# AlanLiangC/PDM-SSD

Measured on AMD Instinct MI355X. Metric: frames/sec (16384-pt clouds, bs=32), higher is better.
Workload: dtype f32; 1 GPU; configs[2]: full PDM-SSD forward (PointNet2MSG backbone + PDM neck + hybrid head: BEV heat-map head + point box head with decoded boxes), bs=32/GPU x 16384 pts, uniform KITTI-range clouds, fp32 inference, inputs resident in HBM, 4 distinct batches in rotation; launch=hipGraph, parallelism=dp1, global_batch=32

## Files before the change

### include/pdmssd_hip.h

```cpp
#ifndef PDMSSD_HIP_H
#define PDMSSD_HIP_H

#include <stddef.h>

#ifdef __cplusplus
extern "C" {
#endif

#define PDM_ABI_VERSION 1

#define PDM_E_BADARG (-1)
#define PDM_E_TOOLARGE (-2)

int pdm_abi_version(void);
const char *pdm_last_error(void);


int pdm_ball_query(void *stream, int b, int n, int m, float radius, int nsample,
                   const float *new_xyz, const float *xyz, int *idx);

int pdm_group_points(void *stream, int b, int c, int n, int npoints, int nsample,
                     const float *points, const int *idx, float *out);

int pdm_group_points_grad(void *stream, int b, int c, int n, int npoints, int nsample,
// ... 339 lines not shown
                            const float *V2C, const float *R0, const float *P2, const int *image_shape, long long capacity,
                            int *out_counts, int *overflow, float *out_rows, void *workspace, size_t workspace_bytes);
int pdm_kitti_data_boxes_count(void *stream, int B, int C, long long total_rows, const float *raw, const int *counts,
                               const float *V2C, const float *R0, const float *P2, const int *image_shape, int M,
                               const float *boxes, const int *box_count, int *num_points_in_gt, int *db_count,
                               long long *totals, void *workspace, size_t workspace_bytes);
int pdm_kitti_data_boxes_fill(void *stream, int B, int C, long long total_rows, const float *raw, const int *counts,
                              const float *V2C, const float *R0, const float *P2, const int *image_shape, int M,
                              const float *boxes, const int *box_count, const double *centres, int *num_points_in_gt,
                              int *db_count, long long *totals, long long capacity_points, long long capacity_entries,
                              float *out_points, long long *out_offsets, float *out_boxes, void *workspace,
                              size_t workspace_bytes);

int pdm_interp_concat_rows(void *stream, int b, int n, int m, int c2, int c1, int ld, const void *known, int known_bf16,
                           const void *skip, int skip_bf16, const int *idx, const float *weight, void *out);
int pdm_interp_concat_rows_grad(void *stream, int b, int n, int m, int c2, int ld, const void *dx, const int *idx,
                                const float *weight, float *dknown, void *workspace, size_t workspace_bytes);
int pdm_interp_concat_rows_grad_out(void *stream, int b, int n, int m, int c2, int ld, const void *dx, const int *idx,
                                    const float *weight, void *dknown, int out_bf16, void *workspace, size_t workspace_bytes);

int pdm_tg_stats_parts(long long rows, int N);
int pdm_tg_gemm_nt(void *stream, long long R, int K, int N, const void *X, long long ldx, const void *W, long long ldw,
                   void *Y, long long ldy, const float *bias, float *stats, const float *x_bn_coef);
int pdm_tg_gemm_nt_dy(void *stream, long long R, int K, int N, const void *dZ, long long lddz, const void *Yp, long long ldyp,
                      const void *W, long long ldw, void *dX, long long lddx, void *dYout, long long lddy, const float *coef,
                      const float *grads);
int pdm_tg_gemm_nt_bs(void *stream, long long R, int K, int N, const void *X, long long ldx, const void *W, long long ldw,
                      void *Y, long long ldy, const void *Bx, long long ldbx, const float *bcoef, float *bstats);
int pdm_tg_gemm_nt_pool(void *stream, long long R, int K, int N, const void *X, long long ldx, const void *W, long long ldw,
                        void *Y, long long ldy, const float *bias, float *stats, const float *x_bn_coef, int ns, void *xmax,
                        void *xmin, unsigned char *imax, unsigned char *imin);
int pdm_tg_dy_stats_parts(long long rows, int N);
int pdm_tg_gemm_nt_dy_bs(void *stream, long long R, int K, int N, const void *dZ, long long lddz, const void *Yp, long long ldyp,
                         const void *W, long long ldw, void *dX, long long lddx, void *dYout, long long lddy, const float *coef,
                         const float *grads, const void *Bx, long long ldbx, const float *bcoef, float *bstats);
size_t pdm_tg_wgrad_ws_bytes(long long R, int K, int N);
int pdm_tg_wgrad(void *stream, long long R, int K, int N, const void *dY, long long ldy, const void *X, long long ldx, float *dW,
                 int accumulate, void *workspace, size_t workspace_bytes, const float *x_bn_coef);
size_t pdm_tg_colsum_ws_floats(long long R, int N);
int pdm_tg_colsum(void *stream, long long R, int N, const void *Y, long long ld, float *out, float *scratch);
int pdm_tg_pack_weight(void *stream, int N, int K, const float *W, void *Wb, int ldb, void *Wt, int ldt);
int pdm_tg_pack_weight_pair(void *stream, int N, int K, const float *W, void *Wb, void *Wt, int rows_to, int cols_to);
int pdm_tg_pack_weight_many(void *stream, int njobs, const void *jobs, long long total_blocks);


int pdm_tune_fps_variant(int v);
int pdm_tune_fused_waves(int w);
int pdm_tune_fused_tiles(int t);
int pdm_tune_fused_groups(int n);
int pdm_tune_fused_wg_per_cu(int n);
int pdm_tune_fused_lds_cap(int bytes);
int pdm_tune_fused_reg(int on);
int pdm_tune_fused_gemm(int on);
int pdm_tune_fused_chain(int on);
int pdm_tune_fused_swz(int on);
int pdm_tune_bq_quad(int form);
int pdm_tune_bq_dense_ppc(int hundredths);
int pdm_tune_grid_split(int min_n);
int pdm_tune_bq_small_waves(int w);
int pdm_tune_bq_cpw(int centres);
int pdm_tune_bq_heavy(int candidates);
int pdm_tune_group_lds_floor(int bytes);
int pdm_tune_group_rows(int packed);
int pdm_tune_rows_chain_wg_per_cu(int n);
int pdm_tune_fp_head_tiles(int n);
int pdm_tune_rows_chain_dw_wg_per_cu(int n);
int pdm_tune_rows_chain_xcd(int on);
int pdm_tune_fp_chain_pad_lds(int bytes);
int pdm_tune_fp_chain_nt(int on);
int pdm_tune_fp_chain_mask(int m);
int pdm_tune_group_nt(int on);
int pdm_tune_copy_variant(int v);
int pdm_tune_copy_max_wg(int n);

int pdm_copy_many(void *stream, int count, void *const *dst, const void *const *src, const size_t *bytes);
int pdm_copy_many_dyn(void *stream, int count, void *const *dst, const void *const *src, const size_t *bytes,
                      const int *const *dyn_count, const unsigned *dyn_unit);


int pdm_scatter_bev(void *stream, int B, int P, int C, int degree, const float *xyz,
                    const float *feat, const float *sh, const float *inv2s2, float ox, float oy,
                    float oz, float cx, float cy, float cz, float icx, float icy, float icz, int W,
                    int H, int D, int kx, int ky, int kz, int layout, float *grid, float *wsum);

int pdm_bev_normalize(void *stream, int B, int C, int W, int H, int D, int layout, float eps,
                      float *grid, const float *wsum);

size_t pdm_gather_bev_workspace_bytes(int B, int P, int W, int H, int kx, int ky);
int pdm_gather_bev(void *stream, int B, int P, int C, int degree, const float *xyz, const float *feat,
                   const float *sh, const float *inv2s2, float ox, float oy, float oz, float cx, float cy,
                   float cz, float icx, float icy, float icz, int W, int H, int D, int kx, int ky, int kz,
                   int normalize, float eps, float *grid, float *wsum, void *workspace, size_t workspace_bytes);

int pdm_bev_normalize_grad(void *stream, int B, int C, int W, int H, int D, float eps, const float *y,
                           const float *wsum, const float *dy, float *dx, float *dwsum);

int pdm_scatter_bev_grad(void *stream, int B, int P, int C, int degree, const float *xyz,
                         const float *feat, const float *sh, const float *inv2s2, float ox,
                         float oy, float oz, float cx, float cy, float cz, float icx, float icy,
                         float icz, int W, int H, int D, int kx, int ky, int kz, int layout,
                         const float *dgrid, const float *dwsum, float *dfeat, float *dsh,
                         float *dinv2s2);
int pdm_scatter_bev_grad_normalized(void *stream, int B, int P, int C, int degree, const float *xyz,
                                    const float *feat, const float *sh, const float *inv2s2, float ox,
                                    float oy, float oz, float cx, float cy, float cz, float icx, float icy,
                                    float icz, int W, int H, int D, int kx, int ky, int kz, int layout,
// ... 67 lines not shown
```

### pdm_ssd_amd/csrc/fused_mlp.hip

```cpp
#include "common.h"

#include <mutex>
#include <set>

namespace pdm {

typedef float f4 __attribute__((ext_vector_type(4)));

constexpr int FM_MAXL = 4;

struct MlpDesc {
    int nlayers;
    int K[FM_MAXL + 1];
    int woff[FM_MAXL];
    int boff[FM_MAXL];
    int stage_in;
    int pool_floats;
    int relu_last;
    int lds_p, lds_q;
    int swz;
};

__device__ __forceinline__ int lds_col(int blk, int g, int pos, int swz) {
    const int q = 4 * blk + g;
// ... 931 lines not shown
    for (int unit = wave_id; unit < npairs; unit += nwaves) {
        f4 in[NT];
        int ctr[NT], L[NT];
#pragma unroll
        for (int t = 0; t < NT; ++t) {
            const int2 e = e_next[t];
            ctr[t] = e.y;
            L[t] = pack_tile_L((unit * 2 + t) * 16, m1, m2, m3, m4, m5);
            in[t] = sa_reg_gather(a, (size_t)e.x, a.new_xyz + (size_t)(e.y >= 0 ? e.y : 0) * 3, g);
        }
        {
            const int nunit = unit + nwaves;
#pragma unroll
            for (int t = 0; t < NT; ++t) e_next[t] = pack[nunit < npairs ? (nunit * 2 + t) * 16 + pos : 0];
        }
        f4 h2[NT][B2];
        sa_reg_hidden<B1, B2, NT>(A1, A2, bias1, bias2, in, h2);
        const bool pair = L[0] >= 32;
        float *orow[NT];
#pragma unroll
        for (int t = 0; t < NT; ++t) {
            const int Lw = L[t] < 16 ? L[t] : 16;
            const bool writer = ctr[t] >= 0 && (pos & (Lw - 1)) == 0 && !(pair && t == 1);
            orow[t] = writer ? a.out + (size_t)ctr[t] * a.out_stride + a.out_coff : nullptr;
        }
#pragma unroll
        for (int mb = 0; mb < B3; ++mb) {
            const f4 bi = *reinterpret_cast<const f4 *>(bias3 + 16 * mb);
            f4 v[NT];
#pragma unroll
            for (int t = 0; t < NT; ++t) {
                f4 acc = bi;
#pragma unroll
                for (int kb = 0; kb < B2; ++kb) acc = mfma4(acc, A3[mb][kb], h2[t][kb]);
                v[t] = floor4(acc, 0.0f);
            }
            if (pair) {
                v[0].x = fmaxf(v[0].x, v[1].x); v[0].y = fmaxf(v[0].y, v[1].y);
                v[0].z = fmaxf(v[0].z, v[1].z); v[0].w = fmaxf(v[0].w, v[1].w);
                v[0] = seg_max_nonneg4(v[0], 16);
            } else {
#pragma unroll
                for (int t = 0; t < NT; ++t) v[t] = seg_max_nonneg4(v[t], L[t]);
            }
#pragma unroll
            for (int t = 0; t < NT; ++t)
                if (orow[t]) sa_reg_store4(orow[t], 16 * mb + 4 * g, a.cout, v[t]);
        }
    }
}

int rows_gemm_launch(void *stream, int rows, int cin, const float *in_pm, int k0, int c1, const float *wpack,
                     const float *bias, int relu_last, float *out_pm, int out_stride, int cout);
int rows_chain_launch(void *stream, int rows, int cin, const float *in_pm, int nlayers, const int *dims, const float *wpack,
                      const float *bias, int relu_last, float *out_pm, int out_stride, int cout, int *launched);
int rows_chain_pair_launch(void *stream, int rows, int cin, const float *in_pm, int nlayers, const int *dims, const float *wpack_a,
                           const float *bias_a, const float *wpack_b, const float *bias_b, int relu_last, float *out_a, int out_stride_a,
                           int cout_a, float *out_b, int out_stride_b, int cout_b, int *launched);
static int g_fused_chain = 1;
static int g_fused_pair = 1;
int fp_chain_launch(void *stream, int b, int n, int m, int c_skip, const float *z_pm, int z_stride, const float *skip_pm,
                    const int *idx, const float *weight, const int *dims, const float *wpack, const float *bias, float *out_pm,
                    int out_stride, int cout, int *launched);
int fp_pre_gemm_launch(void *stream, int b, int n, int m, int c_skip, const float *z_pm, int z_stride,
                       const float *skip_pm, const int *idx, const float *weight, int k1, int c2,
                       const float *wpack, const float *bias, float *out_pm, int out_stride, int cout);
static int g_fused_swz = 1;
static int g_fused_gemm = 1;
static int g_fused_reg = 1;
static int g_fused_waves = 0;
static int g_fused_tiles = 0;
static int g_fused_groups = 0;
static int g_fused_lds_cap = 152 * 1024;
static int g_fused_wg_per_cu = 32;

static int fill_desc(const char *who, MlpDesc &d, int nlayers, const int *dims, int k0_real_max, int pool_floats,
                     long long ntiles, int *waves, int *tiles_per_wg, int *groups, bool two_tiles) {
    PDM_REQUIRE(nlayers >= 1 && nlayers <= FM_MAXL, PDM_E_BADARG, "%s: nlayers=%d not in [1,%d]", who, nlayers, FM_MAXL);
    PDM_REQUIRE(dims, PDM_E_BADARG, "%s: null dims", who);
    d.nlayers = nlayers;
    d.relu_last = 1;
    int wo = 0, bo = 0;
    for (int l = 0; l <= nlayers; ++l) {
        PDM_REQUIRE(dims[l] > 0 && dims[l] % 16 == 0, PDM_E_BADARG, "%s: padded width %d of level %d is not a positive multiple of 16", who, dims[l], l);
        d.K[l] = dims[l];
    }
    for (int l = 0; l < nlayers; ++l) {
        d.woff[l] = wo; d.boff[l] = bo;
        wo += d.K[l] * d.K[l + 1];
        bo += d.K[l + 1];
    }
    PDM_REQUIRE(d.K[0] >= k0_real_max, PDM_E_BADARG, "%s: padded input width %d < %d real channels", who, d.K[0], k0_real_max);
    int q = 0, p = 0;
    for (int l = 1; l < nlayers; ++l) {
        if (l & 1) q = q > d.K[l] ? q : d.K[l]; else p = p > d.K[l] ? p : d.K[l];
    }
    int maxmb = 0;
    for (int l = 1; l <= nlayers; ++l) maxmb = maxmb > (d.K[l] >> 4) ? maxmb : (d.K[l] >> 4);
    const int W = g_fused_waves > 0 ? g_fused_waves : maxmb >= 24 ? 8 : maxmb >= 12 ? 4 : maxmb >= 6 ? 2 : 1;
    *waves = W;
    const int p_staged = p > d.K[0] ? p : d.K[0];
    int NT = (W >= 4 && (g_fused_tiles == 2 || (g_fused_tiles == 0 && two_tiles))) ? 2 : 1;
    (void)ntiles;
    auto roww = [](int k) { return g_fused_swz ? (k + 63) / 64 * 64 : k + 4; };
    if ((NT * 16 * (roww(p) + roww(q)) + pool_floats) * 4 > g_fused_lds_cap) NT = 1;
    *tiles_per_wg = NT;
    const int budget = (W == 1 ? 20 : W == 2 ? 40 : W == 4 ? 52 : 64) * 1024;
    d.stage_in = (NT * 16 * (roww(p_staged) + roww(q)) + pool_floats) * 4 <= budget ? 1 : 0;
    if (d.stage_in) p = p_staged;
    d.swz = g_fused_swz;
    d.lds_p = roww(p);
    d.lds_q = roww(q);
    d.pool_floats = pool_floats;
    const int region_bytes = (NT * 16 * (d.lds_p + d.lds_q) + pool_floats) * 4;
    int G = NT == 2 ? 1 : (g_fused_groups > 0 ? g_fused_groups : W == 2 ? 2 : 1);
    while (G > 1 && (G * W > 8 || (long long)G * region_bytes > 64 * 1024 || (long long)G * NT * 4 > ntiles)) G >>= 1;
    *groups = G;
// ... 202 lines not shown
                "sa_mlp_packed_pair: null table");
    PDM_REQUIRE((pack[0] && meta[0] && pack[1] && meta[1]) || b == 0 || m == 0, PDM_E_BADARG, "sa_mlp_packed_pair: null row list");
    SaPlan pl[2];
    for (int k = 0; k < 2; ++k)
        if (int rc = sa_plan(b, n, m, z_pm ? 0 : cin, nsample[k], xyz, new_xyz, z_pm ? nullptr : feat_pm, z_pm, z_stride, z_coff[k], nullptr,
                             nlayers[k], dims[k], wpack[k], bias[k], out_pm, out_stride, out_coff[k], cout[k], pack[k], meta[k], pl[k])) return rc;
    if (b == 0 || m == 0) return 0;
    const bool same = g_sa_pair && !pl[0].reg && !pl[1].reg && pl[0].W == pl[1].W && pl[0].NT == pl[1].NT && pl[0].G == pl[1].G &&
                      pl[0].pre_form == pl[1].pre_form && pl[0].packed && pl[1].packed;
    if (!same) {
        for (int k = 0; k < 2; ++k)
            if (int rc = pdm_sa_mlp_packed(stream, b, n, m, cin, nsample[k], xyz, new_xyz, feat_pm, z_pm, z_stride, z_coff[k], pack[k], meta[k],
                                           nlayers[k], dims[k], wpack[k], bias[k], out_pm, out_stride, out_coff[k], cout[k])) return rc;
        return 0;
    }
    const int W = pl[0].W, NT = pl[0].NT, G = pl[0].G;
    const bool pre_form = pl[0].pre_form;
    const size_t lds_bytes = pl[0].lds_bytes > pl[1].lds_bytes ? pl[0].lds_bytes : pl[1].lds_bytes;
    const dim3 blocks((unsigned)(pl[0].blocks > pl[1].blocks ? pl[0].blocks : pl[1].blocks), 2);
    const SaScale s0{pl[0].d, pl[0].a, pl[0].pack2, meta[0], wpack[0], bias[0]}, s1{pl[1].d, pl[1].a, pl[1].pack2, meta[1], wpack[1], bias[1]};
    FUSED_DISPATCH(sa_packed_pair_kernel, W, G, blocks, lds_bytes, s0, s1);
    return check_launch("sa_mlp_packed_pair");
}

static int fp_fused_launch(void *stream, int mode, int relu_last, int b, int n, int m, int c_known, int c_skip,
                           const float *known_pm, const float *z_pm, int z_stride, const float *skip_pm,
                           const int *idx, const float *weight, int nlayers, const int *dims,
                           const float *wpack, const float *bias, float *out_pm, int out_stride, int cout) {
    PDM_REQUIRE(b >= 0 && n >= 0 && m >= 1 && c_known >= 0 && c_skip >= 0 && c_known + c_skip >= (mode == 1 ? 0 : 1),
                PDM_E_BADARG, "fp_mlp_fused: bad size");
    if (b == 0 || n == 0) return 0;
    PDM_REQUIRE(wpack && bias && out_pm && (c_skip == 0 || skip_pm) && (mode == 2 || (idx && weight)) &&
                    (mode != 0 || known_pm) && (mode != 1 || z_pm),
                PDM_E_BADARG, "fp_mlp_fused: null pointer");
    MlpDesc d;
    int W = 1, NT = 1, G = 1;
    const long long ntiles = (long long)b * ((n + 15) / 16);
    int rc = fill_desc("fp_mlp_fused", d, nlayers, dims, c_known + c_skip, 0, ntiles, &W, &NT, &G, mode == 1);
    if (rc) return rc;
    d.relu_last = relu_last ? 1 : 0;
    if (mode == 1)
        PDM_REQUIRE(z_stride % 4 == 0 && z_stride >= d.K[1] && (reinterpret_cast<uintptr_t>(z_pm) & 15) == 0, PDM_E_BADARG,
                    "fp_mlp_fused_pre: z rows need %d floats, stride %d, 16-byte aligned", d.K[1], z_stride);
    PDM_REQUIRE(cout > 0 && cout <= d.K[nlayers] && cout <= out_stride, PDM_E_BADARG, "fp_mlp_fused: cout=%d stride=%d", cout, out_stride);
    PDM_REQUIRE(out_stride % 4 == 0 && (reinterpret_cast<uintptr_t>(out_pm) & 15) == 0 &&
                    (reinterpret_cast<uintptr_t>(wpack) & 15) == 0 && (reinterpret_cast<uintptr_t>(bias) & 15) == 0 &&
                    (c_known % 4 != 0 || (reinterpret_cast<uintptr_t>(known_pm) & 15) == 0) &&
                    (c_skip % 4 != 0 || c_skip == 0 || (reinterpret_cast<uintptr_t>(skip_pm) & 15) == 0),
                PDM_E_BADARG, "%s: buffers must be 16-byte aligned and out_stride a multiple of 4",
                mode == 2 ? "rows_mlp_fused" : mode == 1 ? "fp_mlp_fused_pre" : "fp_mlp_fused");
    FpArgs a{b, n, m, c_known, c_skip, known_pm, skip_pm, idx, weight, out_pm, out_stride, cout, mode == 1 ? z_pm : nullptr, z_stride};
    const bool pre_form = mode == 1;
    PDM_REQUIRE(!pre_form || (long long)m * z_stride < (1ll << 31), PDM_E_TOOLARGE, "fp_mlp_fused_pre: m * z_stride overflows 32-bit row offsets");
    if (g_fused_chain && pre_form && nlayers == 2 && z_stride >= d.K[1] &&
        (c_skip <= 4 || (c_skip % 4 == 0 && (reinterpret_cast<uintptr_t>(skip_pm) & 15) == 0))) {
        int launched = 0;
        const int crc = fp_chain_launch(stream, b, n, m, c_skip, z_pm, z_stride, skip_pm, idx, weight, dims, wpack, bias, out_pm,
                                        out_stride, cout, &launched);
        if (crc || launched) return crc;
    }
    if (g_fused_gemm && pre_form && nlayers == 2 && c_skip <= 4 && d.K[0] == 16 && d.K[1] >= 64 && d.K[2] >= 64 &&
        (long long)b * n >= 32768 && (long long)b * n < (1ll << 31) && z_stride >= d.K[1])
        return fp_pre_gemm_launch(stream, b, n, m, c_skip, z_pm, z_stride, skip_pm, idx, weight, d.K[1], d.K[2], wpack, bias,
                                  out_pm, out_stride, cout);
    const size_t lds_bytes = (size_t)G * (NT * 16 * (d.lds_p + d.lds_q)) * sizeof(float);
    PDM_REQUIRE(lds_bytes <= 160 * 1024, PDM_E_TOOLARGE, "fp_mlp_fused: needs %zu bytes of LDS", lds_bytes);
    const long long niter = ((ntiles + NT - 1) / NT + G - 1) / G;
    const long long cap = (long long)256 * g_fused_wg_per_cu;
    const int blocks = (int)(niter < cap ? niter : cap);
    FUSED_DISPATCH(fp_mlp_fused_kernel, W, G, blocks, lds_bytes, d, a, wpack, bias);
    return check_launch("fp_mlp_fused");
}

extern "C" int pdm_fp_mlp_fused(void *stream, int b, int n, int m, int c_known, int c_skip,
                                const float *known_pm, const float *skip_pm, const int *idx,
                                const float *weight, int nlayers, const int *dims, const float *wpack,
                                const float *bias, float *out_pm, int out_stride, int cout) {
    PDM_REQUIRE(c_known >= 1, PDM_E_BADARG, "fp_mlp_fused: c_known=%d", c_known);
    return fp_fused_launch(stream, 0, 1, b, n, m, c_known, c_skip, known_pm, nullptr, 0, skip_pm, idx, weight, nlayers,
                           dims, wpack, bias, out_pm, out_stride, cout);
}

extern "C" int pdm_fp_mlp_fused_pre(void *stream, int b, int n, int m, int c_skip, const float *z_pm,
                                    int z_stride, const float *skip_pm, const int *idx, const float *weight,
                                    int nlayers, const int *dims, const float *wpack, const float *bias,
                                    float *out_pm, int out_stride, int cout) {
    return fp_fused_launch(stream, 1, 1, b, n, m, 0, c_skip, nullptr, z_pm, z_stride, skip_pm, idx, weight, nlayers, dims,
                           wpack, bias, out_pm, out_stride, cout);
}

extern "C" int pdm_rows_mlp_fused(void *stream, int rows, int cin, const float *in_pm, int nlayers,
                                  const int *dims, const float *wpack, const float *bias, int relu_last,
                                  float *out_pm, int out_stride, int cout) {
    PDM_REQUIRE(rows >= 0 && cin >= 1, PDM_E_BADARG, "rows_mlp_fused: rows=%d cin=%d", rows, cin);
    if (g_fused_chain && dims && in_pm && wpack && bias && out_pm && cout > 0 && nlayers >= 1 && nlayers <= 3 && cout <= dims[nlayers] &&
        cout <= out_stride && out_stride % 4 == 0 &&
        ((reinterpret_cast<uintptr_t>(out_pm) | reinterpret_cast<uintptr_t>(wpack) | reinterpret_cast<uintptr_t>(bias) |
          reinterpret_cast<uintptr_t>(in_pm)) & 15) == 0) {
        int launched = 0;
        const int rc = rows_chain_launch(stream, rows, cin, in_pm, nlayers, dims, wpack, bias, relu_last, out_pm, out_stride, cout,
                                         &launched);
        if (rc || launched) return rc;
    }
    if (g_fused_gemm && nlayers == 1 && dims && dims[0] % 16 == 0 && dims[1] % 16 == 0 && dims[0] >= cin && dims[0] >= 32 &&
        dims[1] >= 64 && (long long)((rows + 127) / 128) * ((dims[1] + 127) / 128) >= 256 && in_pm && wpack && bias && out_pm && cout > 0 && cout <= dims[1] && cout <= out_stride &&
        out_stride % 4 == 0 && ((reinterpret_cast<uintptr_t>(out_pm) | reinterpret_cast<uintptr_t>(wpack) |
                                 reinterpret_cast<uintptr_t>(bias)) & 15) == 0)
        return rows_gemm_launch(stream, rows, cin, in_pm, dims[0], dims[1], wpack, bias, relu_last, out_pm, out_stride, cout);
    return fp_fused_launch(stream, 2, relu_last, 1, rows, 1, 0, cin, nullptr, nullptr, 0, in_pm, nullptr, nullptr, nlayers,
                           dims, wpack, bias, out_pm, out_stride, cout);
}

extern "C" int pdm_rows_mlp_fused_pair(void *stream, int rows, int cin, const float *in_pm, int nlayers, const int *dims,
                                       const float *wpack_a, const float *bias_a, const float *wpack_b, const float *bias_b,
                                       int relu_last, float *out_a, int out_stride_a, int cout_a, float *out_b, int out_stride_b,
                                       int cout_b) {
    PDM_REQUIRE(rows >= 0 && cin >= 1, PDM_E_BADARG, "rows_mlp_fused_pair: rows=%d cin=%d", rows, cin);
    if (g_fused_chain && g_fused_pair && dims && in_pm && wpack_a && bias_a && wpack_b && bias_b && out_a && out_b && out_a != out_b &&
        nlayers == 3 && cout_a > 0 && cout_b > 0 && cout_a <= dims[nlayers] && cout_b <= dims[nlayers] && cout_a <= out_stride_a &&
        cout_b <= out_stride_b && out_stride_a % 4 == 0 && out_stride_b % 4 == 0 &&
        ((reinterpret_cast<uintptr_t>(out_a) | reinterpret_cast<uintptr_t>(out_b) | reinterpret_cast<uintptr_t>(wpack_a) |
          reinterpret_cast<uintptr_t>(wpack_b) | reinterpret_cast<uintptr_t>(bias_a) | reinterpret_cast<uintptr_t>(bias_b) |
          reinterpret_cast<uintptr_t>(in_pm)) & 15) == 0) {
        int launched = 0;
        const int rc = rows_chain_pair_launch(stream, rows, cin, in_pm, nlayers, dims, wpack_a, bias_a, wpack_b, bias_b, relu_last, out_a,
                                              out_stride_a, cout_a, out_b, out_stride_b, cout_b, &launched);
        if (rc || launched) return rc;
    }
    if (int rc = pdm_rows_mlp_fused(stream, rows, cin, in_pm, nlayers, dims, wpack_a, bias_a, relu_last, out_a, out_stride_a, cout_a)) return rc;
    return pdm_rows_mlp_fused(stream, rows, cin, in_pm, nlayers, dims, wpack_b, bias_b, relu_last, out_b, out_stride_b, cout_b);
}
```

### pdm_ssd_amd/csrc/rows_gemm.hip

```cpp
#include "common.h"

namespace pdm {

typedef float gf4 __attribute__((ext_vector_type(4)));

constexpr int RG_ROWS = 128;
constexpr int RG_BLKS = 8;
constexpr int RG_HS = 24;

struct RowsGemmArgs {
    int rows, cin, in_stride;
    int nkb, nmb;
    int cout, out_stride;
    const float *in;
    const float *wpack;
    const float *bias;
    float *out;
    float floor;
    int n, m, z_stride, c_skip;
    const float *z;
    const float *skip;
    const int *idx;
    const float *weight;
    const float *w1;
    const float *b1;
};

template <bool FP_PRE>
__global__ __launch_bounds__(512) void rows_gemm_kernel(RowsGemmArgs a) {
    __shared__ __attribute__((aligned(16))) float s_w[2][RG_BLKS * 64 * 4];
    __shared__ __attribute__((aligned(16))) float s_h[2][RG_ROWS * RG_HS];
    const int tid = threadIdx.x, lane = tid & 63;
    const int wave = __builtin_amdgcn_readfirstlane(tid >> 6);
    const int pos = lane & 15, g = lane >> 4;
    const int wp = wave >> 2, wc = wave & 3;
    int tile = blockIdx.x;
    if constexpr (FP_PRE) {
        const int tpc = a.n / RG_ROWS, nb = a.rows / a.n;
        if (gridDim.y == 1 && tpc * RG_ROWS == a.n && (nb & 7) == 0) {
            const int xcd = tile & 7, slot = tile >> 3;
            tile = ((slot / tpc) * 8 + xcd) * tpc + slot % tpc;
        }
    }
    const long long r0 = (long long)tile * RG_ROWS;
    const int mb0 = blockIdx.y * RG_BLKS;

    const int hrow = tid >> 2, part = tid & 3;
    const bool w_live = mb0 + wave < a.nmb;
    const gf4 *wsrc = reinterpret_cast<const gf4 *>(a.wpack) + ((size_t)(mb0 + wave) * a.nkb) * 64 + lane;
    const bool h_live = r0 + hrow < a.rows;
    const float *hsrc = a.in + (size_t)(r0 + hrow) * a.in_stride + 4 * part;
    const bool vec = (a.in_stride & 3) == 0 && (reinterpret_cast<uintptr_t>(a.in) & 15) == 0;

    auto load_w = [&](int kb) {
        gf4 v = {0.f, 0.f, 0.f, 0.f};
        if (w_live) v = wsrc[(size_t)kb * 64];
        return v;
    };
    const float *zb = nullptr;
    int o0 = 0, o1 = 0, o2 = 0;
    float iw0 = 0.f, iw1 = 0.f, iw2 = 0.f, sk[4] = {0.f, 0.f, 0.f, 0.f};
    if constexpr (FP_PRE) {
        if (h_live) {
            const long long row = r0 + hrow;
            const int b = (int)(row / a.n);
            zb = a.z + (size_t)b * a.m * a.z_stride + 4 * part;
            o0 = a.idx[row * 3] * a.z_stride; o1 = a.idx[row * 3 + 1] * a.z_stride; o2 = a.idx[row * 3 + 2] * a.z_stride;
            iw0 = a.weight[row * 3]; iw1 = a.weight[row * 3 + 1]; iw2 = a.weight[row * 3 + 2];
            for (int s_ = 0; s_ < a.c_skip; ++s_) sk[s_] = a.skip[row * a.c_skip + s_];
        }
    }
    struct Raw { gf4 za, zc, zd; };
    auto load_raw = [&](int kb) {
        Raw r;
        r.za = r.zc = r.zd = gf4{0.f, 0.f, 0.f, 0.f};
        if (h_live) {
            r.za = *reinterpret_cast<const gf4 *>(zb + o0 + 16 * kb);
            r.zc = *reinterpret_cast<const gf4 *>(zb + o1 + 16 * kb);
            r.zd = *reinterpret_cast<const gf4 *>(zb + o2 + 16 * kb);
        }
        return r;
    };
    auto finish = [&](const Raw &r, int kb) {
        gf4 v = {0.f, 0.f, 0.f, 0.f};
        if (!h_live) return v;
        const int c = 16 * kb + 4 * part;
        const gf4 bb = *reinterpret_cast<const gf4 *>(a.b1 + c);
        float h[4] = {bb.x, bb.y, bb.z, bb.w};
        const float zz[3][4] = {{r.za.x, r.za.y, r.za.z, r.za.w}, {r.zc.x, r.zc.y, r.zc.z, r.zc.w}, {r.zd.x, r.zd.y, r.zd.z, r.zd.w}};
#pragma unroll
        for (int j = 0; j < 4; ++j) {
            h[j] += __fmaf_rn(iw2, zz[2][j], __fmaf_rn(iw1, zz[1][j], __fmul_rn(iw0, zz[0][j])));
            const float *wr = a.w1 + ((size_t)(c >> 4) * 64 + ((c & 15) + j)) * 4;
            for (int s_ = 0; s_ < a.c_skip; ++s_) h[j] = fmaf(wr[s_], sk[s_], h[j]);
            h[j] = fmaxf(h[j], 0.0f);
        }
        return gf4{h[0], h[1], h[2], h[3]};
    };
    auto load_h = [&](int kb) {
        gf4 v = {0.f, 0.f, 0.f, 0.f};
        if (!h_live) return v;
        const int c = 16 * kb + 4 * part;
        if (vec && c + 4 <= a.cin) return *reinterpret_cast<const gf4 *>(hsrc + 16 * kb);
        const float *p = hsrc + 16 * kb;
        if (c < a.cin) v.x = p[0];
        if (c + 1 < a.cin) v.y = p[1];
        if (c + 2 < a.cin) v.z = p[2];
        if (c + 3 < a.cin) v.w = p[3];
        return v;
    };
    auto stage = [&](int buf, gf4 w, gf4 h) {
        reinterpret_cast<gf4 *>(s_w[buf])[tid] = w;
        *reinterpret_cast<gf4 *>(&s_h[buf][hrow * RG_HS + 4 * part]) = h;
    };

    gf4 acc[2][4];
#pragma unroll
    for (int i = 0; i < 2; ++i) {
        gf4 bi = {0.f, 0.f, 0.f, 0.f};
        if (mb0 + 2 * wc + i < a.nmb) bi = *reinterpret_cast<const gf4 *>(a.bias + 16 * (mb0 + 2 * wc + i) + 4 * g);
#pragma unroll
        for (int t = 0; t < 4; ++t) acc[i][t] = bi;
    }

    gf4 gw = load_w(0), gh = {0.f, 0.f, 0.f, 0.f};
    Raw gr;
    if constexpr (FP_PRE) { gr = load_raw(0); gh = finish(gr, 0); } else gh = load_h(0);
    stage(0, gw, gh);
    __syncthreads();
    if (a.nkb > 1) {
        gw = load_w(1);
        if constexpr (FP_PRE) gr = load_raw(1); else gh = load_h(1);
    }
    for (int kb = 0; kb < a.nkb; ++kb) {
        const int cur = kb & 1;
        gf4 fa[2], fb[4];
#pragma unroll
        for (int i = 0; i < 2; ++i) fa[i] = reinterpret_cast<const gf4 *>(s_w[cur])[(2 * wc + i) * 64 + lane];
#pragma unroll
        for (int t = 0; t < 4; ++t) fb[t] = *reinterpret_cast<const gf4 *>(&s_h[cur][((4 * wp + t) * 16 + pos) * RG_HS + 4 * g]);
        if (kb + 1 < a.nkb) {
            if constexpr (FP_PRE) gh = finish(gr, kb + 1);
            stage(cur ^ 1, gw, gh);
        }
        if (kb + 2 < a.nkb) {
            gw = load_w(kb + 2);
            if constexpr (FP_PRE) gr = load_raw(kb + 2); else gh = load_h(kb + 2);
        }
#define PDM_RG_MFMA(C)                                                                                         \
    _Pragma("unroll") for (int i = 0; i < 2; ++i) _Pragma("unroll") for (int t = 0; t < 4; ++t)                 \
        acc[i][t] = __builtin_amdgcn_mfma_f32_16x16x4f32(fa[i].C, fb[t].C, acc[i][t], 0, 0, 0);
        PDM_RG_MFMA(x) PDM_RG_MFMA(y) PDM_RG_MFMA(z) PDM_RG_MFMA(w)
#undef PDM_RG_MFMA
        __syncthreads();
    }

#pragma unroll
    for (int t = 0; t < 4; ++t) {
        const long long row = r0 + (4 * wp + t) * 16 + pos;
        if (row >= a.rows) continue;
        float *orow = a.out + (size_t)row * a.out_stride;
#pragma unroll
        for (int i = 0; i < 2; ++i) {
            const int c0 = 16 * (mb0 + 2 * wc + i) + 4 * g;
            gf4 v = acc[i][t];
            v.x = __builtin_amdgcn_fmed3f(v.x, a.floor, __builtin_inff()); v.y = __builtin_amdgcn_fmed3f(v.y, a.floor, __builtin_inff());
            v.z = __builtin_amdgcn_fmed3f(v.z, a.floor, __builtin_inff()); v.w = __builtin_amdgcn_fmed3f(v.w, a.floor, __builtin_inff());
            if (c0 + 4 <= a.cout) {
                *reinterpret_cast<gf4 *>(orow + c0) = v;
            } else {
                if (c0 < a.cout) orow[c0] = v.x;
                if (c0 + 1 < a.cout) orow[c0 + 1] = v.y;
                if (c0 + 2 < a.cout) orow[c0 + 2] = v.z;
            }
        }
    }
}

int rows_gemm_launch(void *stream, int rows, int cin, const float *in_pm, int k0, int c1, const float *wpack,
                     const float *bias, int relu_last, float *out_pm, int out_stride, int cout) {
    RowsGemmArgs a;
    a.rows = rows; a.cin = cin; a.in_stride = cin;
    a.nkb = k0 >> 4; a.nmb = c1 >> 4;
    a.cout = cout; a.out_stride = out_stride;
    a.in = in_pm; a.wpack = wpack; a.bias = bias; a.out = out_pm;
    a.floor = relu_last ? 0.0f : -__builtin_inff();
    a.n = a.m = a.z_stride = a.c_skip = 0;
    a.z = a.skip = a.weight = a.w1 = a.b1 = nullptr; a.idx = nullptr;
    const dim3 grid((unsigned)((rows + RG_ROWS - 1) / RG_ROWS), (unsigned)((a.nmb + RG_BLKS - 1) / RG_BLKS));
    hipLaunchKernelGGL(rows_gemm_kernel<false>, grid, dim3(512), 0, as_stream(stream), a);
    return check_launch("rows_mlp_fused(gemm)");
}

int fp_pre_gemm_launch(void *stream, int b, int n, int m, int c_skip, const float *z_pm, int z_stride,
                       const float *skip_pm, const int *idx, const float *weight, int k1, int c2,
                       const float *wpack, const float *bias, float *out_pm, int out_stride, int cout) {
    RowsGemmArgs a;
    a.rows = b * n; a.cin = k1; a.in_stride = 0;
    a.nkb = k1 >> 4; a.nmb = c2 >> 4;
    a.cout = cout; a.out_stride = out_stride;
    a.in = nullptr; a.wpack = wpack + 16 * k1; a.bias = bias + k1; a.out = out_pm;
    a.floor = 0.0f;
    a.n = n; a.m = m; a.z_stride = z_stride; a.c_skip = c_skip;
    a.z = z_pm; a.skip = skip_pm; a.idx = idx; a.weight = weight; a.w1 = wpack; a.b1 = bias;
    const dim3 grid((unsigned)((a.rows + RG_ROWS - 1) / RG_ROWS), (unsigned)((a.nmb + RG_BLKS - 1) / RG_BLKS));
    hipLaunchKernelGGL(rows_gemm_kernel<true>, grid, dim3(512), 0, as_stream(stream), a);
    return check_launch("fp_mlp_fused_pre(gemm)");
}

}
```

Baseline: 7331 frames/s.

## Add 32-deep K staging to rows GEMM with LDS-cached layer-1 weights

Templates the rows GEMM kernel on K-step depth so the FP-pre path can stage 32 channels per pipeline step, halving barriers per K and giving each thread multiple rows. For the deep form, layer-1 bias and skip weights are copied into LDS once per block, and the gather uses global cloud offsets. It also moves to dynamic LDS with a waves-per-EU hint and adds a routing helper plus tuning/route-query entry points. The cost is more LDS and registers per block, which may lower occupancy.

```diff
diff --git a/include/pdmssd_hip.h b/include/pdmssd_hip.h
--- a/include/pdmssd_hip.h
+++ b/include/pdmssd_hip.h
@@ -415,6 +415,8 @@
 int pdm_tune_fused_lds_cap(int bytes);
 int pdm_tune_fused_reg(int on);
 int pdm_tune_fused_gemm(int on);
+int pdm_tune_rows_gemm(int mode);
+int pdm_rows_gemm_route(void);
 int pdm_tune_fused_chain(int on);
 int pdm_tune_fused_swz(int on);
 int pdm_tune_bq_quad(int form);
diff --git a/pdm_ssd_amd/csrc/fused_mlp.hip b/pdm_ssd_amd/csrc/fused_mlp.hip
--- a/pdm_ssd_amd/csrc/fused_mlp.hip
+++ b/pdm_ssd_amd/csrc/fused_mlp.hip
@@ -1007,6 +1007,8 @@
 
 int rows_gemm_launch(void *stream, int rows, int cin, const float *in_pm, int k0, int c1, const float *wpack,
                      const float *bias, int relu_last, float *out_pm, int out_stride, int cout);
+int rows_gemm_form(long long rows, int nmb, int k_floats, long long z_floats, long long min_rows);
+void rows_gemm_note_route(int r);
 int rows_chain_launch(void *stream, int rows, int cin, const float *in_pm, int nlayers, const int *dims, const float *wpack,
                       const float *bias, int relu_last, float *out_pm, int out_stride, int cout, int *launched);
 int rows_chain_pair_launch(void *stream, int rows, int cin, const float *in_pm, int nlayers, const int *dims, const float *wpack_a,
@@ -1017,7 +1019,7 @@
 int fp_chain_launch(void *stream, int b, int n, int m, int c_skip, const float *z_pm, int z_stride, const float *skip_pm,
                     const int *idx, const float *weight, const int *dims, const float *wpack, const float *bias, float *out_pm,
                     int out_stride, int cout, int *launched);
-int fp_pre_gemm_launch(void *stream, int b, int n, int m, int c_skip, const float *z_pm, int z_stride,
+int fp_pre_gemm_launch(void *stream, int form, int b, int n, int m, int c_skip, const float *z_pm, int z_stride,
                        const float *skip_pm, const int *idx, const float *weight, int k1, int c2,
                        const float *wpack, const float *bias, float *out_pm, int out_stride, int cout);
 static int g_fused_swz = 1;
@@ -1326,6 +1328,10 @@
     FpArgs a{b, n, m, c_known, c_skip, known_pm, skip_pm, idx, weight, out_pm, out_stride, cout, mode == 1 ? z_pm : nullptr, z_stride};
     const bool pre_form = mode == 1;
     PDM_REQUIRE(!pre_form || (long long)m * z_stride < (1ll << 31), PDM_E_TOOLARGE, "fp_mlp_fused_pre: m * z_stride overflows 32-bit row offsets");
+    const int gemm_form = g_fused_gemm && pre_form && nlayers == 2 && c_skip <= 4 && d.K[0] == 16 && d.K[1] >= 64 && d.K[2] >= 64 &&
+                                  (long long)b * n < (1ll << 31) && z_stride >= d.K[1]
+                              ? rows_gemm_form((long long)b * n, d.K[2] >> 4, d.K[1], (long long)b * m * z_stride, 32768) : 0;
+    rows_gemm_note_route(0);
     if (g_fused_chain && pre_form && nlayers == 2 && z_stride >= d.K[1] &&
         (c_skip <= 4 || (c_skip % 4 == 0 && (reinterpret_cast<uintptr_t>(skip_pm) & 15) == 0))) {
         int launched = 0;
@@ -1333,10 +1339,9 @@
                                         out_stride, cout, &launched);
         if (crc || launched) return crc;
     }
-    if (g_fused_gemm && pre_form && nlayers == 2 && c_skip <= 4 && d.K[0] == 16 && d.K[1] >= 64 && d.K[2] >= 64 &&
-        (long long)b * n >= 32768 && (long long)b * n < (1ll << 31) && z_stride >= d.K[1])
-        return fp_pre_gemm_launch(stream, b, n, m, c_skip, z_pm, z_stride, skip_pm, idx, weight, d.K[1], d.K[2], wpack, bias,
-                                  out_pm, out_stride, cout);
+    if (gemm_form)
+        return fp_pre_gemm_launch(stream, gemm_form, b, n, m, c_skip, z_pm, z_stride, skip_pm, idx, weight, d.K[1], d.K[2], wpack,
+                                  bias, out_pm, out_stride, cout);
     const size_t lds_bytes = (size_t)G * (NT * 16 * (d.lds_p + d.lds_q)) * sizeof(float);
     PDM_REQUIRE(lds_bytes <= 160 * 1024, PDM_E_TOOLARGE, "fp_mlp_fused: needs %zu bytes of LDS", lds_bytes);
     const long long niter = ((ntiles + NT - 1) / NT + G - 1) / G;
@@ -1367,6 +1372,7 @@
                                   const int *dims, const float *wpack, const float *bias, int relu_last,
                                   float *out_pm, int out_stride, int cout) {
     PDM_REQUIRE(rows >= 0 && cin >= 1, PDM_E_BADARG, "rows_mlp_fused: rows=%d cin=%d", rows, cin);
+    rows_gemm_note_route(0);
     if (g_fused_chain && dims && in_pm && wpack && bias && out_pm && cout > 0 && nlayers >= 1 && nlayers <= 3 && cout <= dims[nlayers] &&
         cout <= out_stride && out_stride % 4 == 0 &&
         ((reinterpret_cast<uintptr_t>(out_pm) | reinterpret_cast<uintptr_t>(wpack) | reinterpret_cast<uintptr_t>(bias) |
@@ -1376,11 +1382,13 @@
                                          &launched);
         if (rc || launched) return rc;
     }
-    if (g_fused_gemm && nlayers == 1 && dims && dims[0] % 16 == 0 && dims[1] % 16 == 0 && dims[0] >= cin && dims[0] >= 32 &&
-        dims[1] >= 64 && (long long)((rows + 127) / 128) * ((dims[1] + 127) / 128) >= 256 && in_pm && wpack && bias && out_pm && cout > 0 && cout <= dims[1] && cout <= out_stride &&
+    if (g_fused_gemm && nlayers == 1 && rows > 0 && dims && dims[0] % 16 == 0 && dims[1] % 16 == 0 && dims[0] >= cin && dims[0] >= 32 &&
+        dims[1] >= 64 && in_pm && wpack && bias && out_pm && cout > 0 && cout <= dims[1] && cout <= out_stride &&
         out_stride % 4 == 0 && ((reinterpret_cast<uintptr_t>(out_pm) | reinterpret_cast<uintptr_t>(wpack) |
-                                 reinterpret_cast<uintptr_t>(bias)) & 15) == 0)
-        return rows_gemm_launch(stream, rows, cin, in_pm, dims[0], dims[1], wpack, bias, relu_last, out_pm, out_stride, cout);
+                                 reinterpret_cast<uintptr_t>(bias)) & 15) == 0) {
+        if (rows_gemm_form(rows, dims[1] >> 4, 0, 0, 0))
+            return rows_gemm_launch(stream, rows, cin, in_pm, dims[0], dims[1], wpack, bias, relu_last, out_pm, out_stride, cout);
+    }
     return fp_fused_launch(stream, 2, relu_last, 1, rows, 1, 0, cin, nullptr, nullptr, 0, in_pm, nullptr, nullptr, nlayers,
                            dims, wpack, bias, out_pm, out_stride, cout);
 }
diff --git a/pdm_ssd_amd/csrc/rows_gemm.hip b/pdm_ssd_amd/csrc/rows_gemm.hip
--- a/pdm_ssd_amd/csrc/rows_gemm.hip
+++ b/pdm_ssd_amd/csrc/rows_gemm.hip
@@ -6,7 +6,8 @@
 
 constexpr int RG_ROWS = 128;
 constexpr int RG_BLKS = 8;
-constexpr int RG_HS = 24;
+template <int BK> constexpr int rg_hs() { return BK == 16 ? 24 : 40; }
+template <int BK> constexpr int rg_stage_floats() { return (BK / 16) * RG_BLKS * 64 * 4 + RG_ROWS * rg_hs<BK>(); }
 
 struct RowsGemmArgs {
     int rows, cin, in_stride;
@@ -26,138 +27,220 @@
     const float *b1;
 };
 
-template <bool FP_PRE>
-__global__ __launch_bounds__(512) void rows_gemm_kernel(RowsGemmArgs a) {
-    __shared__ __attribute__((aligned(16))) float s_w[2][RG_BLKS * 64 * 4];
-    __shared__ __attribute__((aligned(16))) float s_h[2][RG_ROWS * RG_HS];
+template <bool FP_PRE, int BK>
+__global__ __launch_bounds__(512) __attribute__((amdgpu_waves_per_eu(4))) void rows_gemm_kernel(RowsGemmArgs a) {
+    constexpr int KH = BK / 16;
+    constexpr int PARTS = BK / 4;
+    constexpr int ROWS = RG_ROWS;
+    constexpr int NR = ROWS * PARTS / 512;
+    constexpr int NT = ROWS / 32;
+    constexpr int HS = rg_hs<BK>();
+    constexpr int TB = FP_PRE && BK == 32 ? 2 : NT;
+    constexpr int WF = KH * RG_BLKS * 64 * 4, SF = rg_stage_floats<BK>();
+    static_assert(NR >= 1 && NR * 512 == ROWS * PARTS, "tile shape");
+    extern __shared__ __attribute__((aligned(16))) float rg_lds[];
+    auto s_w = [&](int buf) { return rg_lds + buf * SF; };
+    auto s_h = [&](int buf) { return rg_lds + buf * SF + WF; };
     const int tid = threadIdx.x, lane = tid & 63;
     const int wave = __builtin_amdgcn_readfirstlane(tid >> 6);
     const int pos = lane & 15, g = lane >> 4;
     const int wp = wave >> 2, wc = wave & 3;
     int tile = blockIdx.x;
     if constexpr (FP_PRE) {
-        const int tpc = a.n / RG_ROWS, nb = a.rows / a.n;
-        if (gridDim.y == 1 && tpc * RG_ROWS == a.n && (nb & 7) == 0) {
+        const int tpc = a.n / ROWS, nb = a.rows / a.n;
+        if (gridDim.y == 1 && tpc * ROWS == a.n && (nb & 7) == 0) {
             const int xcd = tile & 7, slot = tile >> 3;
             tile = ((slot / tpc) * 8 + xcd) * tpc + slot % tpc;
         }
     }
-    const long long r0 = (long long)tile * RG_ROWS;
+    const long long r0 = (long long)tile * ROWS;
     const int mb0 = blockIdx.y * RG_BLKS;
-
-    const int hrow = tid >> 2, part = tid & 3;
+    const int nst = (a.nkb + KH - 1) / KH;
+
+    const int hrow = tid / PARTS, part = tid % PARTS;
     const bool w_live = mb0 + wave < a.nmb;
     const gf4 *wsrc = reinterpret_cast<const gf4 *>(a.wpack) + ((size_t)(mb0 + wave) * a.nkb) * 64 + lane;
-    const bool h_live = r0 + hrow < a.rows;
-    const float *hsrc = a.in + (size_t)(r0 + hrow) * a.in_stride + 4 * part;
     const bool vec = (a.in_stride & 3) == 0 && (reinterpret_cast<uintptr_t>(a.in) & 15) == 0;
-
-    auto load_w = [&](int kb) {
-        gf4 v = {0.f, 0.f, 0.f, 0.f};
-        if (w_live) v = wsrc[(size_t)kb * 64];
-        return v;
-    };
-    const float *zb = nullptr;
-    int o0 = 0, o1 = 0, o2 = 0;
-    float iw0 = 0.f, iw1 = 0.f, iw2 = 0.f, sk[4] = {0.f, 0.f, 0.f, 0.f};
+    bool h_live[NR];
+    const float *hsrc[NR];
+#pragma unroll
+    for (int q = 0; q < NR; ++q) {
+        const long long row = r0 + hrow + q * (512 / PARTS);
+        h_live[q] = row < a.rows;
+        hsrc[q] = a.in + (size_t)row * a.in_stride + 4 * part;
+    }
+
+    struct W { gf4 v[KH]; };
+    auto load_w = [&](int st) {
+        W w;
+#pragma unroll
+        for (int j = 0; j < KH; ++j) {
+            w.v[j] = gf4{0.f, 0.f, 0.f, 0.f};
+            if (w_live && KH * st + j < a.nkb) w.v[j] = wsrc[(size_t)(KH * st + j) * 64];
+        }
+        return w;
+    };
+    const float *zb[NR];
+    int o0[NR], o1[NR], o2[NR];
+    float iw0[NR], iw1[NR], iw2[NR], sk[NR][4];
     if constexpr (FP_PRE) {
-        if (h_live) {
-            const long long row = r0 + hrow;
-            const int b = (int)(row / a.n);
-            zb = a.z + (size_t)b * a.m * a.z_stride + 4 * part;
-            o0 = a.idx[row * 3] * a.z_stride; o1 = a.idx[row * 3 + 1] * a.z_stride; o2 = a.idx[row * 3 + 2] * a.z_stride;
-            iw0 = a.weight[row * 3]; iw1 = a.weight[row * 3 + 1]; iw2 = a.weight[row * 3 + 2];
-            for (int s_ = 0; s_ < a.c_skip; ++s_) sk[s_] = a.skip[row * a.c_skip + s_];
-        }
-    }
-    struct Raw { gf4 za, zc, zd; };
-    auto load_raw = [&](int kb) {
-        Raw r;
-        r.za = r.zc = r.zd = gf4{0.f, 0.f, 0.f, 0.f};
-        if (h_live) {
-            r.za = *reinterpret_cast<const gf4 *>(zb + o0 + 16 * kb);
-            r.zc = *reinterpret_cast<const gf4 *>(zb + o1 + 16 * kb);
-            r.zd = *reinterpret_cast<const gf4 *>(zb + o2 + 16 * kb);
+#pragma unroll
+        for (int q = 0; q < NR; ++q) {
+            zb[q] = a.z + 4 * part; o0[q] = o1[q] = o2[q] = 0; iw0[q] = iw1[q] = iw2[q] = 0.f;
+            sk[q][0] = sk[q][1] = sk[q][2] = sk[q][3] = 0.f;
+            if (h_live[q]) {
+                const long long row = r0 + hrow + q * (512 / PARTS);
+                const int b = (int)(row / a.n);
+                const int cloud = BK == 32 ? b * a.m : 0;
+                zb[q] = a.z + (BK == 32 ? (size_t)0 : (size_t)b * a.m * a.z_stride) + 4 * part;
+                o0[q] = (cloud + a.idx[row * 3]) * a.z_stride; o1[q] = (cloud + a.idx[row * 3 + 1]) * a.z_stride;
+                o2[q] = (cloud + a.idx[row * 3 + 2]) * a.z_stride;
+                iw0[q] = a.weight[row * 3]; iw1[q] = a.weight[row * 3 + 1]; iw2[q] = a.weight[row * 3 + 2];
+                for (int s_ = 0; s_ < a.c_skip; ++s_) sk[q][s_] = a.skip[row * a.c_skip + s_];
+            }
+        }
+    }
+    struct H { gf4 za[NR], zc[NR], zd[NR]; };
+    auto load_raw = [&](int st) {
+        H r;
+        const int c = BK * st + 4 * part;
+#pragma unroll
+        for (int q = 0; q < NR; ++q) {
+            r.za[q] = r.zc[q] = r.zd[q] = gf4{0.f, 0.f, 0.f, 0.f};
+            if (h_live[q] && c < 16 * a.nkb) {
+                r.za[q] = *reinterpret_cast<const gf4 *>(zb[q] + o0[q] + BK * st);
+                r.zc[q] = *reinterpret_cast<const gf4 *>(zb[q] + o1[q] + BK * st);
+                r.zd[q] = *reinterpret_cast<const gf4 *>(zb[q] + o2[q] + BK * st);
+            }
         }
         return r;
     };
-    auto finish = [&](const Raw &r, int kb) {
-        gf4 v = {0.f, 0.f, 0.f, 0.f};
-        if (!h_live) return v;
-        const int c = 16 * kb + 4 * part;
-        const gf4 bb = *reinterpret_cast<const gf4 *>(a.b1 + c);
-        float h[4] = {bb.x, bb.y, bb.z, bb.w};
-        const float zz[3][4] = {{r.za.x, r.za.y, r.za.z, r.za.w}, {r.zc.x, r.zc.y, r.zc.z, r.zc.w}, {r.zd.x, r.zd.y, r.zd.z, r.zd.w}};
-#pragma unroll
-        for (int j = 0; j < 4; ++j) {
-            h[j] += __fmaf_rn(iw2, zz[2][j], __fmaf_rn(iw1, zz[1][j], __fmul_rn(iw0, zz[0][j])));
-            const float *wr = a.w1 + ((size_t)(c >> 4) * 64 + ((c & 15) + j)) * 4;
-            for (int s_ = 0; s_ < a.c_skip; ++s_) h[j] = fmaf(wr[s_], sk[s_], h[j]);
-            h[j] = fmaxf(h[j], 0.0f);
-        }
-        return gf4{h[0], h[1], h[2], h[3]};
-    };
-    auto load_h = [&](int kb) {
-        gf4 v = {0.f, 0.f, 0.f, 0.f};
-        if (!h_live) return v;
-        const int c = 16 * kb + 4 * part;
-        if (vec && c + 4 <= a.cin) return *reinterpret_cast<const gf4 *>(hsrc + 16 * kb);
-        const float *p = hsrc + 16 * kb;
-        if (c < a.cin) v.x = p[0];
-        if (c + 1 < a.cin) v.y = p[1];
-        if (c + 2 < a.cin) v.z = p[2];
-        if (c + 3 < a.cin) v.w = p[3];
-        return v;
-    };
-    auto stage = [&](int buf, gf4 w, gf4 h) {
-        reinterpret_cast<gf4 *>(s_w[buf])[tid] = w;
-        *reinterpret_cast<gf4 *>(&s_h[buf][hrow * RG_HS + 4 * part]) = h;
-    };
-
-    gf4 acc[2][4];
+    const float *t_b1 = rg_lds + 2 * SF;
+    const gf4 *t_w1 = reinterpret_cast<const gf4 *>(t_b1 + 16 * a.nkb);
+    auto finish = [&](H &r, int st) {
+        const int c = BK * st + 4 * part;
+        if (c >= 16 * a.nkb) return;
+        const gf4 bb = *reinterpret_cast<const gf4 *>((BK == 32 ? t_b1 : a.b1) + c);
+#pragma unroll
+        for (int q = 0; q < NR; ++q) {
+            if (!h_live[q]) continue;
+            float h[4] = {bb.x, bb.y, bb.z, bb.w};
+            const float zz[3][4] = {{r.za[q].x, r.za[q].y, r.za[q].z, r.za[q].w}, {r.zc[q].x, r.zc[q].y, r.zc[q].z, r.zc[q].w},
+                                    {r.zd[q].x, r.zd[q].y, r.zd[q].z, r.zd[q].w}};
+#pragma unroll
+            for (int j = 0; j < 4; ++j) {
+                h[j] += __fmaf_rn(iw2[q], zz[2][j], __fmaf_rn(iw1[q], zz[1][j], __fmul_rn(iw0[q], zz[0][j])));
+                if constexpr (BK == 32) {
+                    const gf4 wr = t_w1[c + j];
+                    const float w4[4] = {wr.x, wr.y, wr.z, wr.w};
+#pragma unroll
+                    for (int s_ = 0; s_ < 4; ++s_)
+                        if (s_ < a.c_skip) h[j] = fmaf(w4[s_], sk[q][s_], h[j]);
+                } else {
+                    const float *wg = a.w1 + ((size_t)(c >> 4) * 64 + ((c & 15) + j)) * 4;
+                    for (int s_ = 0; s_ < a.c_skip; ++s_) h[j] = fmaf(wg[s_], sk[q][s_], h[j]);
+                }
+                h[j] = fmaxf(h[j], 0.0f);
+            }
+            r.za[q] = gf4{h[0], h[1], h[2], h[3]};
+        }
+    };
+    auto load_h = [&](int st) {
+        H r;
+        const int c = BK * st + 4 * part;
+#pragma unroll
+        for (int q = 0; q < NR; ++q) {
+            gf4 v = {0.f, 0.f, 0.f, 0.f};
+            if (h_live[q]) {
+                const float *p = hsrc[q] + BK * st;
+                if (vec && c + 4 <= a.cin) {
+                    v = *reinterpret_cast<const gf4 *>(p);
+                } else {
+                    if (c < a.cin) v.x = p[0];
+                    if (c + 1 < a.cin) v.y = p[1];
+                    if (c + 2 < a.cin) v.z = p[2];
+                    if (c + 3 < a.cin) v.w = p[3];
+                }
+            }
+            r.za[q] = v;
+        }
+        return r;
+    };
+    auto stage = [&](int buf, const W &w, const H &h) {
+#pragma unroll
+        for (int j = 0; j < KH; ++j) reinterpret_cast<gf4 *>(s_w(buf))[j * (RG_BLKS * 64) + tid] = w.v[j];
+#pragma unroll
+        for (int q = 0; q < NR; ++q)
+            *reinterpret_cast<gf4 *>(&s_h(buf)[(hrow + q * (512 / PARTS)) * HS + 4 * part]) = h.za[q];
+    };
+
+    gf4 acc[2][NT];
 #pragma unroll
     for (int i = 0; i < 2; ++i) {
         gf4 bi = {0.f, 0.f, 0.f, 0.f};
         if (mb0 + 2 * wc + i < a.nmb) bi = *reinterpret_cast<const gf4 *>(a.bias + 16 * (mb0 + 2 * wc + i) + 4 * g);
 #pragma unroll
-        for (int t = 0; t < 4; ++t) acc[i][t] = bi;
-    }
-
-    gf4 gw = load_w(0), gh = {0.f, 0.f, 0.f, 0.f};
-    Raw gr;
-    if constexpr (FP_PRE) { gr = load_raw(0); gh = finish(gr, 0); } else gh = load_h(0);
+        for (int t = 0; t < NT; ++t) acc[i][t] = bi;
+    }
+
+    W gw = load_w(0);
+    H gh;
+    if constexpr (FP_PRE) {
+        gh = load_raw(0);
+        if constexpr (BK == 32) {
+            float *tb = rg_lds + 2 * SF;
+            gf4 *tw = reinterpret_cast<gf4 *>(tb + 16 * a.nkb);
+            for (int c = tid; c < 16 * a.nkb; c += 512) {
+                tb[c] = a.b1[c];
+                tw[c] = reinterpret_cast<const gf4 *>(a.w1)[(size_t)(c >> 4) * 64 + (c & 15)];
+            }
+            __syncthreads();
+        }
+        finish(gh, 0);
+    } else {
+        gh = load_h(0);
+    }
     stage(0, gw, gh);
     __syncthreads();
-    if (a.nkb > 1) {
+    if (nst > 1) {
         gw = load_w(1);
-        if constexpr (FP_PRE) gr = load_raw(1); else gh = load_h(1);
-    }
-    for (int kb = 0; kb < a.nkb; ++kb) {
-        const int cur = kb & 1;
-        gf4 fa[2], fb[4];
-#pragma unroll
-        for (int i = 0; i < 2; ++i) fa[i] = reinterpret_cast<const gf4 *>(s_w[cur])[(2 * wc + i) * 64 + lane];
-#pragma unroll
-        for (int t = 0; t < 4; ++t) fb[t] = *reinterpret_cast<const gf4 *>(&s_h[cur][((4 * wp + t) * 16 + pos) * RG_HS + 4 * g]);
-        if (kb + 1 < a.nkb) {
-            if constexpr (FP_PRE) gh = finish(gr, kb + 1);
+        if constexpr (FP_PRE) gh = load_raw(1); else gh = load_h(1);
+    }
+    for (int st = 0; st < nst; ++st) {
+        const int cur = st & 1;
+        if (st + 1 < nst) {
+            if constexpr (FP_PRE) finish(gh, st + 1);
             stage(cur ^ 1, gw, gh);
         }
-        if (kb + 2 < a.nkb) {
-            gw = load_w(kb + 2);
-            if constexpr (FP_PRE) gr = load_raw(kb + 2); else gh = load_h(kb + 2);
-        }
+        if (st + 2 < nst) {
+            gw = load_w(st + 2);
+            if constexpr (FP_PRE) gh = load_raw(st + 2); else gh = load_h(st + 2);
+        }
+#pragma unroll
+        for (int j = 0; j < KH; ++j) {
+            if (j == 1 && 2 * st + 1 >= a.nkb) break;
+            gf4 fa[2];
+#pragma unroll
+            for (int i = 0; i < 2; ++i) fa[i] = reinterpret_cast<const gf4 *>(s_w(cur))[(j * RG_BLKS + 2 * wc + i) * 64 + lane];
+#pragma unroll
+            for (int tb = 0; tb < NT; tb += TB) {
+                gf4 fb[TB];
+#pragma unroll
+                for (int t = 0; t < TB; ++t)
+                    fb[t] = *reinterpret_cast<const gf4 *>(&s_h(cur)[((NT * wp + tb + t) * 16 + pos) * HS + 16 * j + 4 * g]);
 #define PDM_RG_MFMA(C)                                                                                         \
-    _Pragma("unroll") for (int i = 0; i < 2; ++i) _Pragma("unroll") for (int t = 0; t < 4; ++t)                 \
-        acc[i][t] = __builtin_amdgcn_mfma_f32_16x16x4f32(fa[i].C, fb[t].C, acc[i][t], 0, 0, 0);
-        PDM_RG_MFMA(x) PDM_RG_MFMA(y) PDM_RG_MFMA(z) PDM_RG_MFMA(w)
+    _Pragma("unroll") for (int i = 0; i < 2; ++i) _Pragma("unroll") for (int t = 0; t < TB; ++t)                \
+        acc[i][tb + t] = __builtin_amdgcn_mfma_f32_16x16x4f32(fa[i].C, fb[t].C, acc[i][tb + t], 0, 0, 0);
+                PDM_RG_MFMA(x) PDM_RG_MFMA(y) PDM_RG_MFMA(z) PDM_RG_MFMA(w)
+            }
 #undef PDM_RG_MFMA
+        }
         __syncthreads();
     }
 
 #pragma unroll
-    for (int t = 0; t < 4; ++t) {
-        const long long row = r0 + (4 * wp + t) * 16 + pos;
+    for (int t = 0; t < NT; ++t) {
+        const long long row = r0 + (NT * wp + t) * 16 + pos;
         if (row >= a.rows) continue;
         float *orow = a.out + (size_t)row * a.out_stride;
 #pragma unroll
@@ -177,6 +260,31 @@
     }
 }
 
+static int g_rows_gemm = 1;
+static int g_rows_gemm_route = 0;
+void rows_gemm_note_route(int r) { g_rows_gemm_route = r; }
+
+int rows_gemm_form(long long rows, int nmb, int k_floats, long long z_floats, long long min_rows) {
+    const long long tiles = (rows + RG_ROWS - 1) / RG_ROWS * ((nmb + RG_BLKS - 1) / RG_BLKS);
+    const int m = g_rows_gemm;
+    if (m < 2 && (rows < min_rows || (min_rows == 0 && tiles < 256))) return 0;
+    const bool deep = k_floats > 0 && (2 * rg_stage_floats<32>() + 5 * k_floats) * sizeof(float) <= 80 * 1024 && z_floats < (1ll << 31);
+    return deep && (m == 1 || m == 2) ? 32128 : 16128;
+}
+
+template <bool FP_PRE, int BK>
+static int rows_gemm_run(void *stream, const RowsGemmArgs &a, const char *what) {
+    const dim3 grid((unsigned)((a.rows + RG_ROWS - 1) / RG_ROWS), (unsigned)((a.nmb + RG_BLKS - 1) / RG_BLKS));
+    const size_t lds = (2 * rg_stage_floats<BK>() + (FP_PRE && BK == 32 ? 5 * 16 * a.nkb : 0)) * sizeof(float);
+    if (lds > 64 * 1024) {
+        const int e = grant_lds(reinterpret_cast<const void *>(&rows_gemm_kernel<FP_PRE, BK>), 160 * 1024);
+        PDM_REQUIRE(e == 0, PDM_E_TOOLARGE, "%s: cannot obtain %zu bytes of LDS", what, lds);
+    }
+    hipLaunchKernelGGL((rows_gemm_kernel<FP_PRE, BK>), grid, dim3(512), lds, as_stream(stream), a);
+    g_rows_gemm_route = 1000 * BK + RG_ROWS;
+    return check_launch(what);
+}
+
 int rows_gemm_launch(void *stream, int rows, int cin, const float *in_pm, int k0, int c1, const float *wpack,
                      const float *bias, int relu_last, float *out_pm, int out_stride, int cout) {
     RowsGemmArgs a;
@@ -187,12 +295,10 @@
     a.floor = relu_last ? 0.0f : -__builtin_inff();
     a.n = a.m = a.z_stride = a.c_skip = 0;
     a.z = a.skip = a.weight = a.w1 = a.b1 = nullptr; a.idx = nullptr;
-    const dim3 grid((unsigned)((rows + RG_ROWS - 1) / RG_ROWS), (unsigned)((a.nmb + RG_BLKS - 1) / RG_BLKS));
-    hipLaunchKernelGGL(rows_gemm_kernel<false>, grid, dim3(512), 0, as_stream(stream), a);
-    return check_launch("rows_mlp_fused(gemm)");
-}
-
-int fp_pre_gemm_launch(void *stream, int b, int n, int m, int c_skip, const float *z_pm, int z_stride,
+    return rows_gemm_run<false, 16>(stream, a, "rows_mlp_fused(gemm)");
+}
+
+int fp_pre_gemm_launch(void *stream, int form, int b, int n, int m, int c_skip, const float *z_pm, int z_stride,
                        const float *skip_pm, const int *idx, const float *weight, int k1, int c2,
                        const float *wpack, const float *bias, float *out_pm, int out_stride, int cout) {
     RowsGemmArgs a;
@@ -203,9 +309,14 @@
     a.floor = 0.0f;
     a.n = n; a.m = m; a.z_stride = z_stride; a.c_skip = c_skip;
     a.z = z_pm; a.skip = skip_pm; a.idx = idx; a.weight = weight; a.w1 = wpack; a.b1 = bias;
-    const dim3 grid((unsigned)((a.rows + RG_ROWS - 1) / RG_ROWS), (unsigned)((a.nmb + RG_BLKS - 1) / RG_BLKS));
-    hipLaunchKernelGGL(rows_gemm_kernel<true>, grid, dim3(512), 0, as_stream(stream), a);
-    return check_launch("fp_mlp_fused_pre(gemm)");
-}
-
-}
+    return form == 32128 ? rows_gemm_run<true, 32>(stream, a, "fp_mlp_fused_pre(gemm)") : rows_gemm_run<true, 16>(stream, a, "fp_mlp_fused_pre(gemm)");
+}
+
+}
+
+extern "C" int pdm_tune_rows_gemm(int mode) {
+    const int old = pdm::g_rows_gemm;
+    if (mode >= 0 && mode <= 3) pdm::g_rows_gemm = mode;
+    return old;
+}
+extern "C" int pdm_rows_gemm_route(void) { return pdm::g_rows_gemm_route; }
```

Result: no change. 7360 frames/s (median of 2 runs) (+0.4%).
